# fgnt/pb_bss

Hardware: NVIDIA B200
Metric: EM iterations/s, cACGMM F=513 T=500 D=8 K=3 (100-iteration fit) (higher is better)
Workload: dtype f64

## Files before the change

### pb_bss_b200/csrc/api_cacgmm.cu

```cuda
#include <algorithm>
#include <array>
#include <cstdarg>
#include <cstdlib>
#include <cstring>
#include <map>
#include <mutex>
#include <vector>

#include <cuda.h>

#include "em_kernels.cuh"
#include "em_persistent.cuh"
#include "em_ws.cuh"
#include "em_ls.cuh"
#include "em_sticky.cuh"
#include "prof.cuh"

#ifndef PBB_CTA_FPL
#define PBB_CTA_FPL 2
#endif

namespace pbb {

static thread_local char g_err[512] = "";
// ... 31 lines not shown
  const int k = blockIdx.x;
  __shared__ double red[32];
  double s = 0.0;
  for (int t = threadIdx.x; t < T; t += blockDim.x) s += in[(size_t)k * T + t];
  s = warp_sum(s);
  if ((threadIdx.x & 31) == 0) red[threadIdx.x >> 5] = s;
  __syncthreads();
  if (threadIdx.x == 0) {
    double tot = 0.0;
    for (int i = 0; i < (int)(blockDim.x >> 5); ++i) tot += red[i];
    out[k] = tot / (double)T;
  }
}

__global__ void unit_norm_over_classes_kernel(double* __restrict__ w, int K, int T) {
  const int t = blockIdx.x * blockDim.x + threadIdx.x;
  if (t >= T) return;
  double n = 0.0;
  for (int k = 0; k < K; ++k) n += fabs(w[(size_t)k * T + t]);
  if (n == 0.0) n = 1e-10;
  for (int k = 0; k < K; ++k) w[(size_t)k * T + t] /= n;
}

struct CacgmmWorkspace {
  void* z;
  int zs;
  int* flags;
  int* ticket;
  unsigned long long* phase;
  int* dead;
  double* part;
  double* coef;
  double* ld;
  double* w;
  double* ew;
  double* loglik_part;
  double* aff_stage;
  int* tcount;
  size_t bytes;
};

static int max_chunks(int T) { return (T + 31) / 32; }
constexpr int kMaxOrder = 1 << 20;

static CacgmmWorkspace carve(void* base, int F, int T, int D, int K) {
  CacgmmWorkspace ws;
  const size_t NS = (size_t)D * D;
  size_t off = 0;
  auto take = [&](size_t n) { size_t o = off; off += align_up(n); return o; };
  const int zs = (T + 31) / 32 * 32;
  const size_t nchunks = ((size_t)zs + kStageFrames - 1) / kStageFrames;
  const size_t z_plain = (size_t)F * D * zs * sizeof(double2);
  const size_t z_staged = (size_t)F * nchunks * stage_rows(D % 2 == 0 ? D : D + 1) * kStageFrames * sizeof(double2);
  const size_t o_z = take(z_plain > z_staged ? z_plain : z_staged);
  const size_t o_flags = take((size_t)(F + 1) * sizeof(int) + 16 * sizeof(unsigned long long) + 8);
  const size_t o_dead = take((size_t)F * sizeof(int));
  const size_t o_part = take((size_t)F * max_chunks(T) * K * (NS + 1) * sizeof(double));
  const size_t o_coef = take((size_t)F * (K * NS + 8) * sizeof(double));
  const size_t o_ld = take((size_t)F * (K > 4 ? K : 4) * sizeof(double) + 64);
  const size_t o_w = take((size_t)F * K * sizeof(double));
  const size_t o_ew = take((size_t)F * (K > 4 ? K : 4) * sizeof(double) + 64);
  const size_t o_ll = take((size_t)F * max_chunks(T) * sizeof(double));
  const size_t o_aff = take((size_t)F * K * T * sizeof(double));
  const size_t o_tcount = take((size_t)F * sizeof(int));
  char* b = reinterpret_cast<char*>(base);
  ws.z = b + o_z;
  ws.zs = zs;
  ws.flags = reinterpret_cast<int*>(b + o_flags);
  ws.ticket = ws.flags + F;
  ws.dead = reinterpret_cast<int*>(b + o_dead);
  ws.phase = reinterpret_cast<unsigned long long*>(b + o_flags + (((size_t)(F + 1) * sizeof(int) + 7) / 8) * 8);
  ws.part = reinterpret_cast<double*>(b + o_part);
  ws.coef = reinterpret_cast<double*>(b + o_coef);
  ws.ld = reinterpret_cast<double*>(b + o_ld);
  ws.w = reinterpret_cast<double*>(b + o_w);
  ws.ew = reinterpret_cast<double*>(b + o_ew);
  ws.loglik_part = reinterpret_cast<double*>(b + o_ll);
  ws.aff_stage = reinterpret_cast<double*>(b + o_aff);
// ... 530 lines not shown
  {
    bool h = false;
    const void* alias = nullptr;
    if ((r = classify_pointer(eigenvectors, &alias, &h, "eigenvectors"))) return r;
    eigenvectors = const_cast<void*>(alias);
    if ((r = classify_pointer(eigenvalues, &alias, &h, "eigenvalues"))) return r;
    eigenvalues = static_cast<double*>(const_cast<void*>(alias));
    if ((r = classify_pointer(weight, &alias, &h, "weight"))) return r;
    weight = static_cast<double*>(const_cast<void*>(alias));
  }
  const bool streamed = persistent && y_host && init_aff != nullptr && !(opt->reserved & 2) &&
                        ws.aff_stage != nullptr;
  const bool fast_sm = softmax_fast_ok(D, opt);
  const bool lean_ok = fast_sm && (K - 1) * D * (log10(1.0 / opt->eigenvalue_floor) + 1.0) < 290.0;
  const bool full = saliency != nullptr || activity != nullptr || !lean_ok || init_aff == nullptr;
  const int layout = persistent && use_ls_kernel(D, full) ? 1 : 0;
  std::unique_lock<std::mutex> stream_lock;
  if (streamed) {
    LoadStream* lsm = nullptr;
    if ((r = get_load_stream(&lsm))) return r;
    stream_lock = std::unique_lock<std::mutex>(lsm->mu);
  }
  if (streamed) {
    PBB_CUDA(cudaMemsetAsync(ws.flags, 0, (size_t)(F + 1) * sizeof(int) + 16 * sizeof(unsigned long long) + 8, st));
    PBB_CUDA(cudaMemsetAsync(ws.flags, 0xFF, (size_t)F * sizeof(int), st));
    PBB_CUDA(cudaMemsetAsync(ws.dead, 0, (size_t)F * sizeof(int), st));
    LoadStream* l = nullptr;
    if ((r = get_load_stream(&l))) return r;
    PBB_CUDA(cudaEventRecord(l->fork, st));
    PBB_CUDA(cudaStreamWaitEvent(l->stream, l->fork, 0));
    double* aff_dst = aff_host ? ws.aff_stage : nullptr;
    int* next_bin = reinterpret_cast<int*>(ws.phase + 15);
    int* started = reinterpret_cast<int*>(ws.phase + 14);
    int ctas = 0;
    r = dtype == PBB_C128
            ? launch_stream_load<double2>(y, ws.z, init_aff, aff_dst, F, T, D, K, ws.dead, ws.flags, next_bin, started, &ctas, layout, l->stream)
            : launch_stream_load<float2>(y, ws.z, init_aff, aff_dst, F, T, D, K, ws.dead, ws.flags, next_bin, started, &ctas, layout, l->stream);
    if (r) return r;
    PBB_CUDA(cudaEventRecord(l->join, l->stream));
    if (l->wait_value != nullptr) {
      if (l->wait_value(reinterpret_cast<CUstream>(st), reinterpret_cast<CUdeviceptr>(started), (cuuint32_t)ctas,
                        CU_STREAM_WAIT_VALUE_GEQ) != CUDA_SUCCESS)
        l->wait_value = nullptr;
    }
    if (aff_host) init_aff = ws.aff_stage;
  } else if (persistent)
    r = dtype == PBB_C128 ? launch_normalize_staged<double2>(y, ws.z, F, T, D, ws.dead, layout, st)
// ... 5 lines not shown

  EmArgs a;
  memset(&a, 0, sizeof(a));
  a.z = ws.z; a.zs = ws.zs; a.F = F; a.T = T; a.D = D; a.K = K;
  a.coef = ws.coef; a.ld = ws.ld; a.w = ws.w; a.ew = ws.ew;
  a.activity = activity; a.aff_eps = opt->affiliation_eps;
  a.saliency = saliency; a.part = ws.part;

  UpdArgs u;
  memset(&u, 0, sizeof(u));
  u.F = F; u.T = T; u.D = D; u.K = K;
  u.part = ws.part;
  u.covariance_norm = opt->covariance_norm;
  u.weight_mode = opt->weight_mode;
  u.has_saliency = saliency != nullptr;
  u.eigenvalue_floor = opt->eigenvalue_floor;
  u.evec = reinterpret_cast<double2*>(eigenvectors);
  u.eval = eigenvalues; u.weight = weight;
  u.coef = ws.coef; u.ld = ws.ld; u.ew = ws.ew;
  u.status = status;

  if (persistent) {
    if (!streamed)
      PBB_CUDA(cudaMemsetAsync(ws.flags, 0, (size_t)(F + 1) * sizeof(int) + 16 * sizeof(unsigned long long) + 8, st));
    if (init_aff == nullptr) {
      FromEigArgs fe;
      fe.F = F; fe.D = D; fe.K = K;
      fe.evec = reinterpret_cast<const double2*>(eigenvectors);
      fe.eval = eigenvalues; fe.weight = weight;
      fe.coef = ws.coef; fe.ld = ws.ld; fe.w = ws.w; fe.ew = ws.ew;
      if ((r = launch_from_eig(fe, st))) return r;
    }
    PersistArgs p;
    memset(&p, 0, sizeof(p));
    p.z = ws.z; p.zs = ws.zs; p.F = F; p.T = T;
    p.iterations = opt->iterations;
    p.first_is_m = init_aff != nullptr;
    p.user_model = init_aff == nullptr;
    p.softmax_fast = fast_sm;
    p.aff_in = init_aff; p.saliency = saliency; p.activity = activity;
    p.aff_eps = opt->affiliation_eps; p.eigenvalue_floor = opt->eigenvalue_floor;
    p.covariance_norm = opt->covariance_norm; p.weight_mode = opt->weight_mode;
    p.coef = ws.coef; p.ld = ws.ld; p.w = ws.w; p.ew = ws.ew;
    p.part = ws.part; p.flags = ws.flags; p.ticket = ws.ticket; p.status = status;
    p.phase = ws.phase; p.dead = ws.dead;
    if (streamed) {
      const double bin_bytes = (double)T * D * (dtype == PBB_C128 ? 16.0 : 8.0) + (aff_host ? 8.0 * K * T : 0.0);
// ... 10 lines not shown
        PBB_CUDA(cudaDeviceGetAttribute(&sms, cudaDevAttrMultiProcessorCount, dev));
        int cap = (int)(1.6 * (2 * sms - kLoadReserve));
        if (const char* e = getenv("PBB_ORDER_CAP")) cap = atoi(e);
        if ((r = streamed_order(F, opt->iterations, c, cap < 1 ? 1 : cap, &p.order))) return r;
      }
    }
    bool sticky = false;
    if (D == 8 && !full && !streamed && em_kernel_choice() == 1) {
      if ((r = launch_sticky(p, K, dtype, ws.zs, &sticky, st))) return r;
    }
    if (!sticky) {
      if (!(D == 8 && !full && em_kernel_choice() == 0))
        if ((r = setup_frame_split(&p, ws, F, T, D, K, full ? (D == 8 ? 3 : D == 6 ? 4 : 6) : (D == 4 ? 4 : 2), st)))
          return r;
      if ((r = launch_persist(p, D, K, dtype, full, st))) return r;
    }
    if (streamed) {
      LoadStream* l = nullptr;
      if ((r = get_load_stream(&l))) return r;
      PBB_CUDA(cudaStreamWaitEvent(st, l->join, 0));
    }
#ifdef PBB_PHASE_TIMING
    {
      unsigned long long ph[16];
      cudaStreamSynchronize(st);
      cudaMemcpy(ph, ws.phase, sizeof(ph), cudaMemcpyDeviceToHost);
      fprintf(stderr, "[phase] update of class 0, cycles per task: build %.0f  gauss-jordan %.0f  logdet/tinv %.0f  stores %.0f\n",
              ph[8] / (double)((size_t)F * opt->iterations), ph[9] / (double)((size_t)F * opt->iterations),
              ph[10] / (double)((size_t)F * opt->iterations), ph[11] / (double)((size_t)F * opt->iterations));
      fprintf(stderr, "[phase] producer, cycles per task: ticket->dependency %.0f  model buffer wait %.0f  model issue %.0f  ring refill %.0f\n",
              ph[12] / (double)((size_t)F * opt->iterations), ph[13] / (double)((size_t)F * opt->iterations),
              ph[14] / (double)((size_t)F * opt->iterations), ph[15] / (double)((size_t)F * opt->iterations));
      unsigned long long tot = 0;
      for (int i = 0; i < 8; ++i) tot += ph[i];
      static const char* nm[8] = {"ticket+flag / model wait", "chunk-top / updater busy", "tma-wait", "em-steps", "reduce", "update / S wait", "publish / hand-over", "task-start / updater idle"};
      for (int i = 0; i < 8; ++i) fprintf(stderr, "[phase] %-20s %6.2f%%  %8.0f cycles per task\n", nm[i], 100.0 * ph[i] / (double)tot, ph[i] / (double)((size_t)F * opt->iterations));
    }
#endif
    u.nch = 1;
    u.coef = nullptr;
    return launch_update(u, st);
  }
  int it = 0;
  if (init_aff != nullptr) {
    a.mode = kModeM; a.aff_in = init_aff; a.q_in = nullptr;
    int nch = launch_em(a, dtype, opt->frames_per_block, st);
    if (nch <= 0) return nch ? nch : 1;
    u.nch = nch;
    if ((r = launch_update(u, st))) return r;
// ... 128 lines not shown
  int r;
  if (persistent)
    r = dtype == PBB_C128 ? launch_normalize_staged<double2>(y, ws.z, F, T, D, ws.dead, 0, st)
                          : launch_normalize_staged<float2>(y, ws.z, F, T, D, ws.dead, 0, st);
  else
    r = dtype == PBB_C128 ? launch_normalize<double2>(y, ws.z, F, T, D, 1, ws.zs, st)
                          : launch_normalize<float2>(y, ws.z, F, T, D, 1, ws.zs, st);
  if (r) return r;
  EmArgs a;
  memset(&a, 0, sizeof(a));
  a.z = ws.z; a.zs = ws.zs; a.F = F; a.T = T; a.D = D; a.K = K;
  a.model_kind = 1;
  a.coef = ws.coef; a.ld = ws.ld; a.w = weight; a.ew = ws.ew;
  a.saliency = saliency; a.part = ws.part;
  CwUpdArgs u;
  memset(&u, 0, sizeof(u));
  u.F = F; u.T = T; u.D = D; u.K = K;
  u.part = ws.part; u.weight_mode = weight_mode;
  u.spline.t = spline_t; u.spline.c = spline_c; u.spline.n = spline_n;
  u.spline.max_concentration = max_concentration;
  u.mode = reinterpret_cast<double2*>(mode); u.concentration = concentration; u.weight = weight;
  u.coef = ws.coef; u.ld = ws.ld; u.ew = ws.ew; u.status = status;
  if (persistent) {
    PBB_CUDA(cudaMemsetAsync(ws.flags, 0, (size_t)(F + 1) * sizeof(int) + 16 * sizeof(unsigned long long) + 8, st));
    PersistArgs p;
    memset(&p, 0, sizeof(p));
    p.z = ws.z; p.zs = ws.zs; p.F = F; p.T = T;
    p.iterations = iterations; p.first_is_m = 1; p.user_model = 0; p.softmax_fast = 0;
    p.aff_in = init_aff; p.aff_eps = 0.0; p.weight_mode = weight_mode;
    p.coef = ws.coef; p.ld = ws.ld; p.w = ws.w; p.ew = ws.ew;
    p.part = ws.part; p.flags = ws.flags; p.ticket = ws.ticket; p.status = status; p.phase = ws.phase;
    p.spline = u.spline;
    if ((r = setup_frame_split(&p, ws, F, T, D, K, D == 4 ? 4 : 2, st))) return r;
    if ((r = launch_persist_cw(p, D, K, dtype, st))) return r;
#ifdef PBB_PHASE_TIMING
    {
      unsigned long long ph[16];
      cudaStreamSynchronize(st);
      cudaMemcpy(ph, ws.phase, sizeof(ph), cudaMemcpyDeviceToHost);
      unsigned long long tot = 0;
      for (int i = 0; i < 8; ++i) tot += ph[i];
      static const char* nm[8] = {"flag wait", "chunk top / staging", "tma-wait", "em-steps", "reduce", "update (jacobi)", "publish", "task-start"};
      for (int i = 0; i < 8; ++i) fprintf(stderr, "[phase cw] %-20s %6.2f%%  %8.0f cycles per task\n", nm[i], 100.0 * ph[i] / (double)tot, ph[i] / (double)((size_t)F * iterations));
    }
#endif
    u.nch = 1;
    return launch_cw_update(u, st);
// ... 73 lines not shown
```

### pb_bss_b200/csrc/em_ls.cuh

```cuda
#pragma once
#include "em_ws.cuh"

namespace pbb {

constexpr int kLsWarps = 8;
constexpr int kLsHelpers = 4;
constexpr int kLsThreads = 32 * (kLsWarps + kLsHelpers);
constexpr int kLsUnit = 32;
#ifndef PBB_LS_REGS
#define PBB_LS_REGS 96
#endif
constexpr int kLsRegs = PBB_LS_REGS;
constexpr int kLsHelperRegs = (384 * 80 - 256 * PBB_LS_REGS) / 128;
constexpr int kLsSmemBudget = 113 * 1024;
#ifndef PBB_LS_LEAD
#define PBB_LS_LEAD 0
#endif
#ifndef PBB_LS_HELPERS_FIRST
#define PBB_LS_HELPERS_FIRST 1
#endif

__host__ __device__ constexpr int ls_chan(int h, int r) {
  return h == 0 ? r : (r < 4 ? 4 + r : ((r - 4 + 1) & 3));
}
// ... 521 lines not shown
        int t = 0;
        if (lane == 0) t = atomicAdd(a.ticket, 1);
        t = __shfl_sync(0xffffffffu, t, 0);
        int bin = -1, it = 0;
        if (t < total) {
          if (a.order != nullptr) {
            const int v = __ldcg(a.order + t);
            bin = v & 0xffff;
            it = v >> 16;
          } else {
            decode_ticket(t, F, a.iterations, a.wave_c, bin, it);
          }
        }
        const bool mstep_only = a.first_is_m && it == 0;
        const bool late_z = mstep_only && a.wait_load;
        int dead_bin = 0;
        if (bin >= 0 && a.dead != nullptr && !late_z) dead_bin = __ldcg(a.dead + bin);
        int issued = 0;
        auto issue_chunks = [&](int upto, bool blocking) {
          while (issued < upto) {
            const int st = chunk_cnt % STAGES;
            const uint32_t par = ((chunk_cnt / STAGES) & 1u) ^ 1u;
            if (blocking) {
              mbar_wait_relaxed(&sm.empty[st], par, 100);
            } else {
              uint32_t done;
              asm volatile(
                  "{\n"
                  ".reg .pred p;\n"
                  "mbarrier.test_wait.parity.shared::cta.b64 p, [%1], %2;\n"
                  "selp.u32 %0, 1, 0, p;\n"
                  "}\n"
                  : "=r"(done)
                  : "r"(smem_u32(&sm.empty[st])), "r"(par)
                  : "memory");
              if (!done) break;
            }
            mbar_expect_tx(&sm.full[st], kStageBytes);
            bulk_g2s(&sm.zbuf[st][0][0], zbase + ((size_t)bin * nchunks + issued) * (kStageFrames * 8), kStageBytes,
                     &sm.full[st]);
            ++chunk_cnt;
            ++issued;
          }
        };
#ifdef PBB_PHASE_TIMING
        long long _pt = clock64();
#define PBB_PP(i) do { if (lane == 0) { long long _t = clock64(); atomicAdd(&a.phase[i], (unsigned long long)(_t - _pt)); _pt = _t; } } while (0)
#else
#define PBB_PP(i) do { } while (0)
#endif
        if (bin >= 0 && lane == 0) {
          if (!late_z) issue_chunks(nchunks, false);
          if (mstep_only) {
            if (a.wait_load) while (ld_acquire_gpu(a.flags + bin) < 0) __nanosleep(200);
          } else {
            while (ld_acquire_gpu(a.flags + bin) < it) {
              issue_chunks(nchunks, false);
              __nanosleep(40);
            }
          }
          if (late_z) asm volatile("fence.proxy.async;" ::: "memory");
        }
        __syncwarp();
        PBB_PP(12);
        mbar_wait_relaxed(&sm.model_empty[mb], ((n >> 1) & 1u) ^ 1u, 100);
        PBB_PP(13);
        if (late_z && a.dead != nullptr) dead_bin = __ldcg(a.dead + bin);
        if (bin >= 0 && !mstep_only) {
          constexpr int kPieces = ls_model_doubles(K) / 2;
          constexpr int kRounds = (kPieces + 31) / 32;
          const double2* __restrict__ src = reinterpret_cast<const double2*>(a.coef + (size_t)bin * ls_model_doubles(K));
          double2* __restrict__ dst = reinterpret_cast<double2*>(&sm.model[mb]);
          double2 v[kRounds];
#pragma unroll
          for (int r = 0; r < kRounds; ++r)
            if (lane + 32 * r < kPieces) v[r] = __ldcg(src + lane + 32 * r);
#pragma unroll
          for (int r = 0; r < kRounds; ++r)
            if (lane + 32 * r < kPieces) dst[lane + 32 * r] = v[r];
        }
        if (lane == 0) {
          sm.desc[mb][0] = bin;
          sm.desc[mb][1] = it;
          sm.desc[mb][2] = dead_bin;
        }
        __syncwarp();
        if (lane == 0) mbar_arrive(&sm.model_full[mb]);
        if (bin < 0) break;
        PBB_PP(14);
        if (lane == 0) {
          issue_chunks(nchunks, true);
#if PBB_LS_LEAD
          const unsigned x = chunk_cnt - (unsigned)nchunks;
          mbar_wait_relaxed(&sm.empty[x % STAGES], (x / STAGES) & 1u, 100);
#endif
        }
        __syncwarp();
        PBB_PP(15);
      }
    } else if (hw - 1 < NU) {
      const int u = hw - 1;
      int em[2];
#pragma unroll
      for (int r = 0; r < 2; ++r) {
        const int i = (lane >> 3) + 4 * r, c = lane & 7;
        if (i == c) {
          em[r] = ls_diag_slot(i) | 256;
        } else {
          bool rev = false;
          const int sl = ls_pair_slot(i, c, &rev);
          em[r] = sl | (rev ? 1024 : 512);
        }
      }
#ifdef PBB_PHASE_TIMING
      long long _tp = clock64();
#undef PBB_PH
#define PBB_PH(i) do { if (u == 0 && lane == 0) { long long _t = clock64(); atomicAdd(&a.phase[i], (unsigned long long)(_t - _tp)); _tp = _t; } } while (0)
#endif
#pragma unroll 1
      for (unsigned n = 0;; ++n) {
        mbar_wait_relaxed(&sm.s_full, n & 1u, 100);
        PBB_PH(7);
        const int bin = sm.sdesc[0], it = sm.sdesc[1], dead_bin = sm.sdesc[2];
        if (bin < 0) break;
        const bool last_it = it == a.iterations - 1;
        const int par = n & 1;
        for (int k = u; k < K; k += NU) {
          for (int s = lane; s < NS + 1; s += 32) {
            double v[kLsWarps];
#pragma unroll
            for (int w = 0; w < kLsWarps; ++w) v[w] = sm.Spart[w][k][s];
            sm.S[k][s] = ((v[0] + v[1]) + (v[2] + v[3])) + ((v[4] + v[5]) + (v[6] + v[7]));
          }
        }
        __syncwarp();
        if (lane == 0) mbar_arrive(&sm.s_empty);
        if (last_it) {
          asm volatile("bar.sync 2, %0;" ::"n"(NU * 32) : "memory");
          double* __restrict__ po = a.part + (size_t)bin * K * (NS + 1);
          for (int i = u * 32 + lane; i < K * (NS + 1); i += NU * 32) po[i] = (&sm.S[0][0])[i];
          asm volatile("bar.sync 2, %0;" ::"n"(NU * 32) : "memory");
        } else {
          const bool plain = a.covariance_norm != PBB_NORM_NONE && dead_bin == 0;
          for (int k = u; k < K; k += NU) {
// ... 29 lines not shown
```

### pb_bss_b200/csrc/em_persistent.cuh

```cuda
#pragma once
#include "common.cuh"
#include "em_kernels.cuh"
#include "heig.cuh"

namespace pbb {

#ifdef PBB_PHASE_TIMING
#define PBB_PH(i) do { if (tid == 0) { long long _t = clock64(); atomicAdd(&a.phase[i], (unsigned long long)(_t - _tp)); _tp = _t; } } while (0)
#else
#define PBB_PH(i) do { } while (0)
#endif

struct PersistArgs {
  const void* z;
  int zs;
  int F, T;
  int iterations;
  int first_is_m;
  int user_model;
  int softmax_fast;
  const double* aff_in;
  const double* saliency;
  const uint8_t* activity;
  double aff_eps;
  double eigenvalue_floor;
  int covariance_norm;
  int weight_mode;
  double* coef;
  double* ld;
  double* w;
  double* ew;
  double* part;
  int* flags;
  int* ticket;
  const int* dead;
  int* status;
  CwSpline spline;
  int wave_c;
  int wait_load;
  const int* order;
  unsigned long long* phase;
  int tsplit;
  double* tpart;
  int* tcount;
};

__device__ __forceinline__ uint32_t smem_u32(const void* p) {
  return static_cast<uint32_t>(__cvta_generic_to_shared(p));
}
__device__ __forceinline__ void mbar_init(uint64_t* bar, int count) {
  asm volatile("mbarrier.init.shared::cta.b64 [%0], %1;" ::"r"(smem_u32(bar)), "r"(count) : "memory");
}
__device__ __forceinline__ void mbar_expect_tx(uint64_t* bar, uint32_t bytes) {
  asm volatile("mbarrier.arrive.expect_tx.shared::cta.b64 _, [%0], %1;" ::"r"(smem_u32(bar)), "r"(bytes)
               : "memory");
}
__device__ __forceinline__ void mbar_wait(uint64_t* bar, uint32_t parity) {
  asm volatile(
      "{\n"
      ".reg .pred p;\n"
      "WAIT_%=:\n"
      "mbarrier.try_wait.parity.shared::cta.b64 p, [%0], %1;\n"
      "@p bra DONE_%=;\n"
      "bra WAIT_%=;\n"
      "DONE_%=:\n"
      "}\n" ::"r"(smem_u32(bar)),
      "r"(parity)
      : "memory");
}
__device__ __forceinline__ void bulk_g2s(void* dst, const void* src, uint32_t bytes, uint64_t* bar) {
  asm volatile("cp.async.bulk.shared::cluster.global.mbarrier::complete_tx::bytes [%0], [%1], %2, [%3];" ::"r"(
                   smem_u32(dst)),
               "l"(src), "r"(bytes), "r"(smem_u32(bar))
               : "memory");
}
__device__ __forceinline__ int ld_acquire_gpu(const int* p) {
  int v;
  asm volatile("ld.acquire.gpu.global.s32 %0, [%1];" : "=r"(v) : "l"(p) : "memory");
  return v;
}
__device__ __forceinline__ void st_release_gpu(int* p, int v) {
  asm volatile("st.release.gpu.global.s32 [%0], %1;" ::"l"(p), "r"(v) : "memory");
}
__device__ __forceinline__ double fast_rcp(double x) {
  double r;
  asm("rcp.approx.ftz.f64 %0, %1;" : "=d"(r) : "d"(x));
  double e = fma(-x, r, 1.0);
  r = fma(r, e, r);
  e = fma(-x, r, 1.0);
  r = fma(r, e, r);
  return r;
// ... 455 lines not shown
        done = true;
      }
    }
    if (!done) {
#pragma unroll
      for (int k = 0; k < K; ++k) {
        gam[k] = __ldcg(a.aff_in + ((size_t)bin * K + k) * T + tc);
        invq[k] = 1.0;
      }
    }
    double sal = 1.0;
    if (FULL && a.saliency != nullptr) sal = a.saliency[(size_t)bin * T + tc];
#pragma unroll
    for (int k = 0; k < K; ++k) {
      const double gs = valid ? gam[k] * sal : 0.0;
      const double cw = gs * invq[k];
      sg[k] += gs;
#pragma unroll
      for (int i = 0; i < NSG; ++i) acc[k * NSG + i] = fma(cw, psi[i], acc[k * NSG + i]);
    }
  }
}

template <int D>
__device__ __forceinline__ double warp_hpd_inverse(double2* __restrict__ A, int lane, bool* ok) {
  constexpr int NS = D * D;
  constexpr int PER = (NS + 31) / 32;
  int ri[PER], ci[PER];
  double2 mine[PER];
#pragma unroll
  for (int r = 0; r < PER; ++r) {
    const int idx = lane + 32 * r;
    ri[r] = idx / D;
    ci[r] = idx - ri[r] * D;
    mine[r] = idx < NS ? A[idx] : make_double2(0.0, 0.0);
  }
  double det = 1.0;
  bool good = true;
#pragma unroll 1
  for (int j = 0; j < D; ++j) {
    const double p = A[j * D + j].x;
    good = good && (p > 0.0) && (p < 1e300);
    const double ip = fast_rcp(p);
    det *= p;
#pragma unroll
    for (int r = 0; r < PER; ++r) {
      if (lane + 32 * r < NS) {
        const int i = ri[r], k = ci[r];
// ... 52 lines not shown
        else if (kind == 1) { Ad[2 * (d * D + e)] = v; Ad[2 * (e * D + d)] = v; }
        else { Ad[2 * (d * D + e) + 1] = -v; Ad[2 * (e * D + d) + 1] = v; }
      }
      __syncwarp();
    };
    auto build = [&]() { build_scaled(scale); };
    double tr, tn;
    if (a.covariance_norm == PBB_NORM_NONE) {
      build();
      tr = 0.0;
      for (int d = lane; d < D; d += 32) tr += A[d * D + d].x;
      tr = warp_sum(tr);
      tn = 1.0;
    } else {
      double trs = 0.0;
#pragma unroll
      for (int d = 0; d < D; ++d) trs += Sk[(d >> 1) * (NS / (D / 2)) + (d & 1)];
      tr = trs * scale;
      tn = (double)D / fmax(tr, kTiny);
      build_scaled(scale * tn);
    }
    PBB_PHU(8);
    bool ok;
    const double det = warp_hpd_inverse<D>(A, lane, &ok);
    PBB_PHU(9);
    double ldk = log(det);
    double tinv = 0.0;
#pragma unroll
    for (int d = 0; d < D; ++d) tinv += A[d * D + d].x;
    const bool no_floor = ok && isfinite(tinv) && (tr * tn * tinv * a.eigenvalue_floor < 0.5) &&
                          dead_bin == 0;
    double* __restrict__ co = coef_out != nullptr ? coef_out
                              : LS ? a.coef + (size_t)bin * ls_model_doubles(K) : a.coef + ((size_t)bin * K + k) * NS;
    PBB_PHU(10);
    if (__any_sync(0xffffffffu, bad)) {
      if (lane == 0) atomicMax(a.status, bin + 1);
    }
    if (no_floor) {
      for (int s = lane; s < NS; s += 32) {
        const int pk = tab[s];
        const int d = pk & 255, e = (pk >> 8) & 255, kind = pk >> 16;
        const double2 u = A[d * D + e], v = A[e * D + d];
        const double cv = kind == 0 ? u.x : (kind == 1 ? (u.x + v.x) : -(u.y - v.y));
        if constexpr (LS) ls_store_coef(co, tabE, K, k, s, cv);
        else co[s] = cv;
      }
    } else {
// ... 392 lines not shown
```

### pb_bss_b200/csrc/em_ws.cuh

```cuda
#pragma once
#include "em_persistent.cuh"

namespace pbb {

#ifndef PBB_NO_SOFTMAX_SPLIT
#define PBB_SOFTMAX_SPLIT 1
#endif
#ifndef PBB_WS_LEAD
#define PBB_WS_LEAD 2
#endif
constexpr int kWsStages = 3;
#ifndef PBB_WS_EM_REGS
#define PBB_WS_EM_REGS 208
#endif
constexpr int kWsEmRegs = PBB_WS_EM_REGS;
constexpr int kWsHelperRegs = 256 - PBB_WS_EM_REGS;

__device__ __forceinline__ void mbar_arrive(uint64_t* bar) {
  asm volatile("mbarrier.arrive.shared::cta.b64 _, [%0];" ::"r"(smem_u32(bar)) : "memory");
}

__device__ __forceinline__ void mbar_wait_relaxed(uint64_t* bar, uint32_t parity, unsigned ns) {
  while (true) {
    uint32_t done;
    asm volatile(
        "{\n"
        ".reg .pred p;\n"
        "mbarrier.try_wait.parity.shared::cta.b64 p, [%1], %2;\n"
        "selp.u32 %0, 1, 0, p;\n"
        "}\n"
        : "=r"(done)
        : "r"(smem_u32(bar)), "r"(parity)
        : "memory");
    if (done) break;
    __nanosleep(ns);
  }
}

template <int D, int K, typename CT>
struct WsSmem {
  static constexpr int NS = D * D;
  static constexpr int M = D / 2;
  static constexpr int ROWS = stage_rows(D);
  CT zbuf[kWsStages][ROWS][kStageFrames];
  double2 A[K][NS];
  double2 V[K][NS];
  double coef[2][K][NS];
  double xq[2][M][2 * K][32];
  double cwx[K][64];
  double sgp[2][M][K];
  double S[2][K][NS + 1];
  double lam[K][D];
  double ld[K];
  alignas(16) double ew[2][4];
  int tab[NS];
  int desc[2][4];
  int sdesc[2][4];
  int tlast;
  uint64_t full[kWsStages], empty[kWsStages];
  uint64_t model_full[2], model_empty[2];
// ... 14 lines not shown
  const int nchunks = (zs + kStageFrames - 1) / kStageFrames;
  const int S = a.tsplit > 1 ? a.tsplit : 1;
  const int total = a.iterations * F * S;
  constexpr uint32_t kStageBytes = (uint32_t)(SM::ROWS * kStageFrames * sizeof(CT));

  for (int s = tid; s < NS; s += blockDim.x) sm.tab[s] = slot_pack(D, s);
  if (tid == 0) {
    for (int s = 0; s < kWsStages; ++s) { mbar_init(&sm.full[s], 1); mbar_init(&sm.empty[s], M); }
    for (int s = 0; s < 2; ++s) {
      mbar_init(&sm.model_full[s], 1);
      mbar_init(&sm.model_empty[s], M);
      mbar_init(&sm.s_full[s], M);
      mbar_init(&sm.s_empty[s], NU);
    }
    asm volatile("fence.mbarrier_init.release.cluster;" ::: "memory");
  }
  __syncthreads();

  if (warp < M) {
    asm volatile("setmaxnreg.inc.sync.aligned.u32 %0;" ::"n"(kWsEmRegs));
    const int g = warp;
    unsigned chunk_cnt = 0;
    int buf = 0;
#ifdef PBB_PHASE_TIMING
    long long _tp = clock64();
#endif
#pragma unroll 1
    for (unsigned n = 0;; ++n) {
      const int mb = n & 1;
      mbar_wait(&sm.model_full[mb], (n >> 1) & 1u);
      PBB_PH(0);
      const int bin = sm.desc[mb][0], it = sm.desc[mb][1], part = sm.desc[mb][2];
      const int c0 = part * nchunks / S, c1 = (part + 1) * nchunks / S;
      if (bin < 0) {
        const int sb = n & 1;
        mbar_wait(&sm.s_empty[sb], ((n >> 1) & 1u) ^ 1u);
        if (lane == 0) {
          if (g == 0) sm.sdesc[sb][0] = -1;
          mbar_arrive(&sm.s_full[sb]);
        }
        break;
      }
      const bool mstep_only = a.first_is_m && it == 0;
      double acc[K * NSG];
#pragma unroll
      for (int i = 0; i < K * NSG; ++i) acc[i] = 0.0;
      double sg[K];
#pragma unroll
      for (int k = 0; k < K; ++k) sg[k] = 0.0;
#pragma unroll 1
      for (int c = c0; c < c1; ++c) {
        const int st = chunk_cnt % kWsStages;
        mbar_wait(&sm.full[st], (chunk_cnt / kWsStages) & 1u);
        PBB_PH(2);
        const int t_chunk = c * kStageFrames;
        const int nsteps = (min(kStageFrames, zs - t_chunk)) >> 5;
        if (!mstep_only) {
#ifdef PBB_SOFTMAX_SPLIT
          lean_chunk2_split<D, K, CT>(sm, mb, g, st, nsteps >> 1, lane, a.aff_eps, acc, sg);
          if (nsteps & 1) {
            double sgt[K];
#pragma unroll
            for (int k = 0; k < K; ++k) sgt[k] = 0.0;
            buf = 0;
            lean_chunk<D, K, CT, MODEL, true>(sm, mb, g, st, 1, lane, buf, a.aff_eps, acc, sgt, nsteps - 1);
#pragma unroll
            for (int k = 0; k < K; ++k) sg[k] += g == 0 ? sgt[k] : 0.0;
          }
#else
          lean_chunk2<D, K, CT, MODEL, true>(sm, mb, g, st, nsteps >> 1, lane, buf, a.aff_eps, acc, sg);
          if (nsteps & 1) lean_chunk<D, K, CT, MODEL, true>(sm, mb, g, st, 1, lane, buf, a.aff_eps, acc, sg, nsteps - 1);
#endif
        } else {
          general_chunk<D, K, CT, false>(a, sm, g, bin, st, t_chunk, nsteps, lane, buf, true, true, acc, sg);
        }
        __syncwarp();
// ... 6 lines not shown
#pragma unroll
        for (int k = 0; k < K; ++k) q1[k] = 0.0;
        softmax_product<D, K>(q1, sm.ew[mb], a.aff_eps, gp, cp);
#ifdef PBB_SOFTMAX_SPLIT
        const int npad_lane = (g == 0 && lane >= 32 - (zs - T)) ? 1 : 0;
#else
        const int npad_lane = (lane >= 32 - (zs - T)) ? 1 : 0;
#endif
#pragma unroll
        for (int k = 0; k < K; ++k) sg[k] -= npad_lane ? gp[k] : 0.0;
      }
#ifdef PBB_SOFTMAX_SPLIT
      if (mstep_only && g != 0) {
#pragma unroll
        for (int k = 0; k < K; ++k) sg[k] = 0.0;
      }
#endif
      __syncwarp();
      if (lane == 0) mbar_arrive(&sm.model_empty[mb]);

      warp_reduce_halving<K * NSG>(acc, lane);
      const int sb = n & 1;
      PBB_PH(4);
      mbar_wait(&sm.s_empty[sb], ((n >> 1) & 1u) ^ 1u);
      PBB_PH(5);
      {
        int lo, hi;
        reduce_range<K * NSG>(lane, lo, hi);
#pragma unroll
        for (int j = 0; j < HalvingSizes<K * NSG>::n5; ++j) {
          const int idx = lo + j;
          if (idx < hi) {
            const int k = idx / NSG, i = idx - k * NSG;
            sm.S[sb][k][g * NSG + i] = acc[j];
          }
        }
      }
#pragma unroll
      for (int k = 0; k < K; ++k) {
        const double v = warp_sum(sg[k]);
#ifdef PBB_SOFTMAX_SPLIT
        if (lane == 0) sm.sgp[sb][g][k] = v;
#else
        if (g == 0 && lane == 0) sm.S[sb][k][NS] = v;
#endif
      }
      if (g == 0 && lane == 0) { sm.sdesc[sb][0] = bin; sm.sdesc[sb][1] = it; sm.sdesc[sb][2] = part; }
      __syncwarp();
      if (lane == 0) mbar_arrive(&sm.s_full[sb]);
      PBB_PH(6);
    }
  } else {
    asm volatile("setmaxnreg.dec.sync.aligned.u32 %0;" ::"n"(kWsHelperRegs));
    if (warp == M) {
      const CT* __restrict__ zbase = reinterpret_cast<const CT*>(a.z);
      unsigned chunk_cnt = 0;
#pragma unroll 1
      for (unsigned n = 0;; ++n) {
        const int mb = n & 1;
        int t = 0;
        if (lane == 0) t = atomicAdd(a.ticket, 1);
        t = __shfl_sync(0xffffffffu, t, 0);
        int bin = -1, it = 0, part = 0;
        if (t < total) {
          const int tt = t / S;
          part = t - tt * S;
          if (a.order != nullptr) {
            const int v = __ldcg(a.order + tt);
            bin = v & 0xffff;
            it = v >> 16;
          } else {
            decode_ticket(tt, F, a.iterations, a.wave_c, bin, it);
          }
        }
        const int c0 = part * nchunks / S, ncp = (part + 1) * nchunks / S - c0;
        const bool mstep_only = a.first_is_m && it == 0;
        const bool late_z = mstep_only && a.wait_load;
        int issued = 0;
        auto issue_chunks = [&](int upto, bool blocking) {
          while (issued < upto) {
            const int st = chunk_cnt % kWsStages;
            const uint32_t par = ((chunk_cnt / kWsStages) & 1u) ^ 1u;
            if (blocking) {
              mbar_wait_relaxed(&sm.empty[st], par, 100);
            } else {
              uint32_t done;
              asm volatile(
                  "{\n"
                  ".reg .pred p;\n"
                  "mbarrier.test_wait.parity.shared::cta.b64 p, [%1], %2;\n"
                  "selp.u32 %0, 1, 0, p;\n"
                  "}\n"
                  : "=r"(done)
                  : "r"(smem_u32(&sm.empty[st])), "r"(par)
                  : "memory");
              if (!done) break;
            }
            mbar_expect_tx(&sm.full[st], kStageBytes);
            bulk_g2s(&sm.zbuf[st][0][0], zbase + ((size_t)bin * nchunks + c0 + issued) * (SM::ROWS * kStageFrames),
                     kStageBytes, &sm.full[st]);
            ++chunk_cnt;
            ++issued;
          }
        };
        if (bin >= 0 && lane == 0) {
          if (!late_z) issue_chunks(ncp, false);
          if (mstep_only) {
            if (a.wait_load) while (ld_acquire_gpu(a.flags + bin) < 0) __nanosleep(200);
          } else {
            while (ld_acquire_gpu(a.flags + bin) < it) {
              issue_chunks(ncp, false);
              __nanosleep(40);
            }
          }
          if (late_z) asm volatile("fence.proxy.async;" ::: "memory");
        }
        __syncwarp();
        mbar_wait_relaxed(&sm.model_empty[mb], ((n >> 1) & 1u) ^ 1u, 100);
        if (bin >= 0 && !mstep_only) {
          const double* __restrict__ cf = a.coef + (size_t)bin * K * NS;
          for (int i = lane; i < K * NS; i += 32) (&sm.coef[mb][0][0])[i] = __ldcg(cf + i);
          if (lane < K) {
            const double ldk = __ldcg(a.ld + (size_t)bin * 4 + lane);
            double ldmin = ldk;
#pragma unroll
            for (int j = 0; j < K; ++j) ldmin = fmin(ldmin, __ldcg(a.ld + (size_t)bin * 4 + j));
            const double sgam = __ldcg(a.ew + (size_t)bin * 4 + lane);
            const double wk = a.weight_mode == PBB_WEIGHT_CONST ? 1.0 / K : sgam / (double)T;
            sm.ew[mb][lane] = wk * exp(ldmin - ldk);
          }
        }
        if (lane == 0) { sm.desc[mb][0] = bin; sm.desc[mb][1] = it; sm.desc[mb][2] = part; }
        __syncwarp();
        if (lane == 0) mbar_arrive(&sm.model_full[mb]);
        if (bin < 0) break;
        if (lane == 0) {
          issue_chunks(ncp, true);
          const unsigned x = chunk_cnt - (unsigned)(ncp >= PBB_WS_LEAD + 1 ? PBB_WS_LEAD + 1 : ncp);
          mbar_wait_relaxed(&sm.empty[x % kWsStages], (x / kWsStages) & 1u, 100);
        }
        __syncwarp();
      }
    } else if (warp - M - 1 < NU) {
      const int u = warp - M - 1;
#ifdef PBB_PHASE_TIMING
      long long _tp = clock64();
#undef PBB_PH
#define PBB_PH(i) do { if (u == 0 && lane == 0) { long long _t = clock64(); atomicAdd(&a.phase[i], (unsigned long long)(_t - _tp)); _tp = _t; } } while (0)
#endif
#pragma unroll 1
      for (unsigned n = 0;; ++n) {
        const int sb = n & 1;
        mbar_wait_relaxed(&sm.s_full[sb], (n >> 1) & 1u, 100);
        PBB_PH(7);
        const int bin = sm.sdesc[sb][0], it = sm.sdesc[sb][1];
        if (bin < 0) break;
        const bool last_it = it == a.iterations - 1;
#ifdef PBB_SOFTMAX_SPLIT
        for (int k = u; k < K; k += NU)
          if (lane == 0)
            sm.S[sb][k][NS] = (sm.sgp[sb][0][k] + sm.sgp[sb][1][k]) + (sm.sgp[sb][2][k] + sm.sgp[sb][3][k]);
        __syncwarp();
        if (last_it && S == 1) asm volatile("bar.sync 2, %0;" ::"n"(NU * 32) : "memory");
#endif
        if (S > 1) {
          const int part = sm.sdesc[sb][2];
          constexpr int kRow = K * (NS + 1);
          double* __restrict__ tp = a.tpart + ((size_t)bin * S + part) * kRow;
          for (int k = u; k < K; k += NU)
            for (int i = lane; i < NS + 1; i += 32) __stcg(tp + k * (NS + 1) + i, sm.S[sb][k][i]);
          __threadfence();
          asm volatile("bar.sync 2, %0;" ::"n"(NU * 32) : "memory");
          if (u == 0 && lane == 0) {
            const int old = atomicAdd(a.tcount + bin, 1);
            __threadfence();
            sm.tlast = (old + 1 == (it + 1) * S);
          }
          asm volatile("bar.sync 2, %0;" ::"n"(NU * 32) : "memory");
          if (!sm.tlast) {
// ... 35 lines not shown
```

Baseline: 43600.

## Use hinted mbarrier waits, backoff flag polling, and block 8x8 HPD inverse

Replaces the sleep-based mbarrier polling in helper warps with try_wait carrying a suspend-time hint, so threads park in hardware instead of spinning with fixed nanosleeps. The load-flag poll now backs off exponentially instead of sleeping a fixed interval. It also adds a specialised 2x2-block Gauss-Jordan inverse for D=8 that ping-pongs between two shared buffers, plus trip-count instrumentation that only compiles under the phase-timing flag. Long hint values could delay wakeups in helper warps if the hardware honours the full suspend window.

```diff
diff --git a/pb_bss_b200/csrc/api_cacgmm.cu b/pb_bss_b200/csrc/api_cacgmm.cu
--- a/pb_bss_b200/csrc/api_cacgmm.cu
+++ b/pb_bss_b200/csrc/api_cacgmm.cu
@@ -77,6 +77,7 @@
   for (int k = 0; k < K; ++k) w[(size_t)k * T + t] /= n;
 }
 
+constexpr int kPhaseSlots = 32;
 struct CacgmmWorkspace {
   void* z;
   int zs;
@@ -108,7 +109,7 @@
   const size_t z_plain = (size_t)F * D * zs * sizeof(double2);
   const size_t z_staged = (size_t)F * nchunks * stage_rows(D % 2 == 0 ? D : D + 1) * kStageFrames * sizeof(double2);
   const size_t o_z = take(z_plain > z_staged ? z_plain : z_staged);
-  const size_t o_flags = take((size_t)(F + 1) * sizeof(int) + 16 * sizeof(unsigned long long) + 8);
+  const size_t o_flags = take((size_t)(F + 1) * sizeof(int) + kPhaseSlots * sizeof(unsigned long long) + 8);
   const size_t o_dead = take((size_t)F * sizeof(int));
   const size_t o_part = take((size_t)F * max_chunks(T) * K * (NS + 1) * sizeof(double));
   const size_t o_coef = take((size_t)F * (K * NS + 8) * sizeof(double));
@@ -685,7 +686,7 @@
     stream_lock = std::unique_lock<std::mutex>(lsm->mu);
   }
   if (streamed) {
-    PBB_CUDA(cudaMemsetAsync(ws.flags, 0, (size_t)(F + 1) * sizeof(int) + 16 * sizeof(unsigned long long) + 8, st));
+    PBB_CUDA(cudaMemsetAsync(ws.flags, 0, (size_t)(F + 1) * sizeof(int) + kPhaseSlots * sizeof(unsigned long long) + 8, st));
     PBB_CUDA(cudaMemsetAsync(ws.flags, 0xFF, (size_t)F * sizeof(int), st));
     PBB_CUDA(cudaMemsetAsync(ws.dead, 0, (size_t)F * sizeof(int), st));
     LoadStream* l = nullptr;
@@ -737,7 +738,7 @@
 
   if (persistent) {
     if (!streamed)
-      PBB_CUDA(cudaMemsetAsync(ws.flags, 0, (size_t)(F + 1) * sizeof(int) + 16 * sizeof(unsigned long long) + 8, st));
+      PBB_CUDA(cudaMemsetAsync(ws.flags, 0, (size_t)(F + 1) * sizeof(int) + kPhaseSlots * sizeof(unsigned long long) + 8, st));
     if (init_aff == nullptr) {
       FromEigArgs fe;
       fe.F = F; fe.D = D; fe.K = K;
@@ -794,9 +795,14 @@
     }
 #ifdef PBB_PHASE_TIMING
     {
-      unsigned long long ph[16];
+      unsigned long long ph[kPhaseSlots];
       cudaStreamSynchronize(st);
       cudaMemcpy(ph, ws.phase, sizeof(ph), cudaMemcpyDeviceToHost);
+      static const char* tn[7] = {"EM model", "EM ring", "EM S buffer", "producer ring slot", "producer flag poll",
+                                  "producer model buffer", "updater S buffer"};
+      for (int i = 0; i < 7; ++i)
+        fprintf(stderr, "[trips] %-22s %10llu  %8.2f per task\n", tn[i], ph[kPhaseTrip + i],
+                ph[kPhaseTrip + i] / (double)((size_t)F * opt->iterations));
       fprintf(stderr, "[phase] update of class 0, cycles per task: build %.0f  gauss-jordan %.0f  logdet/tinv %.0f  stores %.0f\n",
               ph[8] / (double)((size_t)F * opt->iterations), ph[9] / (double)((size_t)F * opt->iterations),
               ph[10] / (double)((size_t)F * opt->iterations), ph[11] / (double)((size_t)F * opt->iterations));
@@ -971,7 +977,7 @@
   u.mode = reinterpret_cast<double2*>(mode); u.concentration = concentration; u.weight = weight;
   u.coef = ws.coef; u.ld = ws.ld; u.ew = ws.ew; u.status = status;
   if (persistent) {
-    PBB_CUDA(cudaMemsetAsync(ws.flags, 0, (size_t)(F + 1) * sizeof(int) + 16 * sizeof(unsigned long long) + 8, st));
+    PBB_CUDA(cudaMemsetAsync(ws.flags, 0, (size_t)(F + 1) * sizeof(int) + kPhaseSlots * sizeof(unsigned long long) + 8, st));
     PersistArgs p;
     memset(&p, 0, sizeof(p));
     p.z = ws.z; p.zs = ws.zs; p.F = F; p.T = T;
diff --git a/pb_bss_b200/csrc/em_ls.cuh b/pb_bss_b200/csrc/em_ls.cuh
--- a/pb_bss_b200/csrc/em_ls.cuh
+++ b/pb_bss_b200/csrc/em_ls.cuh
@@ -567,7 +567,7 @@
             const int st = chunk_cnt % STAGES;
             const uint32_t par = ((chunk_cnt / STAGES) & 1u) ^ 1u;
             if (blocking) {
-              mbar_wait_relaxed(&sm.empty[st], par, 100);
+              mbar_wait(&sm.empty[st], par, kWaitHintHelper);
             } else {
               uint32_t done;
               asm volatile(
@@ -608,7 +608,7 @@
         }
         __syncwarp();
         PBB_PP(12);
-        mbar_wait_relaxed(&sm.model_empty[mb], ((n >> 1) & 1u) ^ 1u, 100);
+        mbar_wait(&sm.model_empty[mb], ((n >> 1) & 1u) ^ 1u, kWaitHintHelper);
         PBB_PP(13);
         if (late_z && a.dead != nullptr) dead_bin = __ldcg(a.dead + bin);
         if (bin >= 0 && !mstep_only) {
@@ -637,7 +637,7 @@
           issue_chunks(nchunks, true);
 #if PBB_LS_LEAD
           const unsigned x = chunk_cnt - (unsigned)nchunks;
-          mbar_wait_relaxed(&sm.empty[x % STAGES], (x / STAGES) & 1u, 100);
+          mbar_wait(&sm.empty[x % STAGES], (x / STAGES) & 1u, kWaitHintHelper);
 #endif
         }
         __syncwarp();
@@ -664,7 +664,7 @@
 #endif
 #pragma unroll 1
       for (unsigned n = 0;; ++n) {
-        mbar_wait_relaxed(&sm.s_full, n & 1u, 100);
+        mbar_wait(&sm.s_full, n & 1u, kWaitHintHelper);
         PBB_PH(7);
         const int bin = sm.sdesc[0], it = sm.sdesc[1], dead_bin = sm.sdesc[2];
         if (bin < 0) break;
diff --git a/pb_bss_b200/csrc/em_persistent.cuh b/pb_bss_b200/csrc/em_persistent.cuh
--- a/pb_bss_b200/csrc/em_persistent.cuh
+++ b/pb_bss_b200/csrc/em_persistent.cuh
@@ -7,8 +7,15 @@
 
 #ifdef PBB_PHASE_TIMING
 #define PBB_PH(i) do { if (tid == 0) { long long _t = clock64(); atomicAdd(&a.phase[i], (unsigned long long)(_t - _tp)); _tp = _t; } } while (0)
+constexpr int kPhaseTrip = 16;
+#define PBB_TRIPS_DECL(n) unsigned long long _trips[n] = {}; constexpr int _ntrips = n
+#define PBB_TRIP(j, e) (_trips[j] += (e))
+#define PBB_TRIPS_FLUSH(base) do { if (lane == 0) for (int _j = 0; _j < _ntrips; ++_j) atomicAdd(&a.phase[(base) + _j], _trips[_j]); } while (0)
 #else
 #define PBB_PH(i) do { } while (0)
+#define PBB_TRIPS_DECL(n) do { } while (0)
+#define PBB_TRIP(j, e) ((void)(e))
+#define PBB_TRIPS_FLUSH(base) do { } while (0)
 #endif
 
 struct PersistArgs {
@@ -55,18 +62,25 @@
   asm volatile("mbarrier.arrive.expect_tx.shared::cta.b64 _, [%0], %1;" ::"r"(smem_u32(bar)), "r"(bytes)
                : "memory");
 }
-__device__ __forceinline__ void mbar_wait(uint64_t* bar, uint32_t parity) {
+__device__ __forceinline__ bool mbar_try_wait(uint64_t* bar, uint32_t parity, uint32_t hint_ns) {
+  uint32_t done;
   asm volatile(
       "{\n"
       ".reg .pred p;\n"
-      "WAIT_%=:\n"
-      "mbarrier.try_wait.parity.shared::cta.b64 p, [%0], %1;\n"
-      "@p bra DONE_%=;\n"
-      "bra WAIT_%=;\n"
-      "DONE_%=:\n"
-      "}\n" ::"r"(smem_u32(bar)),
-      "r"(parity)
+      "mbarrier.try_wait.parity.shared::cta.b64 p, [%1], %2, %3;\n"
+      "selp.u32 %0, 1, 0, p;\n"
+      "}\n"
+      : "=r"(done)
+      : "r"(smem_u32(bar)), "r"(parity), "r"(hint_ns)
       : "memory");
+  return done != 0;
+}
+constexpr uint32_t kWaitHintEm = 2000;
+constexpr uint32_t kWaitHintHelper = 1000000;
+__device__ __forceinline__ unsigned mbar_wait(uint64_t* bar, uint32_t parity, uint32_t hint_ns = kWaitHintEm) {
+  unsigned trips = 1;
+  while (!mbar_try_wait(bar, parity, hint_ns)) ++trips;
+  return trips;
 }
 __device__ __forceinline__ void bulk_g2s(void* dst, const void* src, uint32_t bytes, uint64_t* bar) {
   asm volatile("cp.async.bulk.shared::cluster.global.mbarrier::complete_tx::bytes [%0], [%1], %2, [%3];" ::"r"(
@@ -568,8 +582,67 @@
   }
 }
 
+__device__ __forceinline__ double2 cfma(double2 y, double2 b, double2 acc) {
+  return make_double2(fma(y.x, b.x, fma(-y.y, b.y, acc.x)), fma(y.x, b.y, fma(y.y, b.x, acc.y)));
+}
+
+__device__ __forceinline__ double warp_hpd_inverse8(double2* __restrict__ A, double2* __restrict__ W, int lane,
+                                                    bool* ok) {
+  constexpr int D = 8;
+  const int i = lane >> 2, c = lane & 3, I = i >> 1, r0 = i & 1;
+  double2 m0 = A[i * D + 2 * c], m1 = A[i * D + 2 * c + 1];
+  double det = 1.0;
+  bool good = true;
+#pragma unroll
+  for (int j = 0; j < 4; ++j) {
+    const double2* __restrict__ src = (j & 1) ? W : A;
+    double2* __restrict__ dst = (j & 1) ? A : W;
+    const int p = 2 * j;
+    const double pa = src[p * D + p].x, pd = src[(p + 1) * D + p + 1].x;
+    const double2 pb = src[p * D + p + 1];
+    const double dp = fma(pa, pd, -fma(pb.x, pb.x, pb.y * pb.y));
+    good = good && (pa > 0.0) && (dp > 0.0) && (pa < 1e300) && (dp < 1e300);
+    det *= dp;
+    const double r = fast_rcp(dp);
+    const double ia = pd * r, id = pa * r;
+    const double2 ib = make_double2(-pb.x * r, -pb.y * r);
+    double2 y0, y1;
+    if (I == j) {
+      y0 = r0 ? make_double2(ib.x, -ib.y) : make_double2(ia, 0.0);
+      y1 = r0 ? make_double2(id, 0.0) : ib;
+    } else {
+      const double2 x0 = src[i * D + p], x1 = src[i * D + p + 1];
+      y0 = make_double2(fma(x0.x, ia, fma(x1.x, ib.x, x1.y * ib.y)), fma(x0.y, ia, fma(x1.y, ib.x, -x1.x * ib.y)));
+      y1 = make_double2(fma(x0.x, ib.x, fma(-x0.y, ib.y, x1.x * id)), fma(x0.x, ib.y, fma(x0.y, ib.x, x1.y * id)));
+    }
+    if (c == j) {
+      m0 = I == j ? y0 : make_double2(-y0.x, -y0.y);
+      m1 = I == j ? y1 : make_double2(-y1.x, -y1.y);
+    } else {
+      const double2 b00 = src[p * D + 2 * c], b01 = src[p * D + 2 * c + 1];
+      const double2 b10 = src[(p + 1) * D + 2 * c], b11 = src[(p + 1) * D + 2 * c + 1];
+      if (I == j) {
+        m0 = make_double2(0.0, 0.0);
+        m1 = make_double2(0.0, 0.0);
+      } else {
+        y0 = make_double2(-y0.x, -y0.y);
+        y1 = make_double2(-y1.x, -y1.y);
+      }
+      m0 = cfma(y1, b10, cfma(y0, b00, m0));
+      m1 = cfma(y1, b11, cfma(y0, b01, m1));
+    }
+    dst[i * D + 2 * c] = m0;
+    dst[i * D + 2 * c + 1] = m1;
+    __syncwarp();
+  }
+  *ok = good;
+  return det;
+}
+
 template <int D>
-__device__ __forceinline__ double warp_hpd_inverse(double2* __restrict__ A, int lane, bool* ok) {
+__device__ __forceinline__ double warp_hpd_inverse(double2* __restrict__ A, double2* __restrict__ W, int lane,
+                                                   bool* ok) {
+  if constexpr (D == 8) return warp_hpd_inverse8(A, W, lane, ok);
   constexpr int NS = D * D;
   constexpr int PER = (NS + 31) / 32;
   int ri[PER], ci[PER];
@@ -668,7 +741,7 @@
     }
     PBB_PHU(8);
     bool ok;
-    const double det = warp_hpd_inverse<D>(A, lane, &ok);
+    const double det = warp_hpd_inverse<D>(A, V, lane, &ok);
     PBB_PHU(9);
     double ldk = log(det);
     double tinv = 0.0;
diff --git a/pb_bss_b200/csrc/em_ws.cuh b/pb_bss_b200/csrc/em_ws.cuh
--- a/pb_bss_b200/csrc/em_ws.cuh
+++ b/pb_bss_b200/csrc/em_ws.cuh
@@ -20,22 +20,7 @@
   asm volatile("mbarrier.arrive.shared::cta.b64 _, [%0];" ::"r"(smem_u32(bar)) : "memory");
 }
 
-__device__ __forceinline__ void mbar_wait_relaxed(uint64_t* bar, uint32_t parity, unsigned ns) {
-  while (true) {
-    uint32_t done;
-    asm volatile(
-        "{\n"
-        ".reg .pred p;\n"
-        "mbarrier.try_wait.parity.shared::cta.b64 p, [%1], %2;\n"
-        "selp.u32 %0, 1, 0, p;\n"
-        "}\n"
-        : "=r"(done)
-        : "r"(smem_u32(bar)), "r"(parity)
-        : "memory");
-    if (done) break;
-    __nanosleep(ns);
-  }
-}
+constexpr unsigned kFlagPollMinNs = 32, kFlagPollMaxNs = 256;
 
 template <int D, int K, typename CT>
 struct WsSmem {
@@ -96,23 +81,25 @@
     const int g = warp;
     unsigned chunk_cnt = 0;
     int buf = 0;
+    PBB_TRIPS_DECL(3);
 #ifdef PBB_PHASE_TIMING
     long long _tp = clock64();
 #endif
 #pragma unroll 1
     for (unsigned n = 0;; ++n) {
       const int mb = n & 1;
-      mbar_wait(&sm.model_full[mb], (n >> 1) & 1u);
+      PBB_TRIP(0, mbar_wait(&sm.model_full[mb], (n >> 1) & 1u));
       PBB_PH(0);
       const int bin = sm.desc[mb][0], it = sm.desc[mb][1], part = sm.desc[mb][2];
       const int c0 = part * nchunks / S, c1 = (part + 1) * nchunks / S;
       if (bin < 0) {
         const int sb = n & 1;
-        mbar_wait(&sm.s_empty[sb], ((n >> 1) & 1u) ^ 1u);
+        PBB_TRIP(2, mbar_wait(&sm.s_empty[sb], ((n >> 1) & 1u) ^ 1u));
         if (lane == 0) {
           if (g == 0) sm.sdesc[sb][0] = -1;
           mbar_arrive(&sm.s_full[sb]);
         }
+        PBB_TRIPS_FLUSH(kPhaseTrip);
         break;
       }
       const bool mstep_only = a.first_is_m && it == 0;
@@ -125,7 +112,7 @@
 #pragma unroll 1
       for (int c = c0; c < c1; ++c) {
         const int st = chunk_cnt % kWsStages;
-        mbar_wait(&sm.full[st], (chunk_cnt / kWsStages) & 1u);
+        PBB_TRIP(1, mbar_wait(&sm.full[st], (chunk_cnt / kWsStages) & 1u));
         PBB_PH(2);
         const int t_chunk = c * kStageFrames;
         const int nsteps = (min(kStageFrames, zs - t_chunk)) >> 5;
@@ -178,7 +165,7 @@
       warp_reduce_halving<K * NSG>(acc, lane);
       const int sb = n & 1;
       PBB_PH(4);
-      mbar_wait(&sm.s_empty[sb], ((n >> 1) & 1u) ^ 1u);
+      PBB_TRIP(2, mbar_wait(&sm.s_empty[sb], ((n >> 1) & 1u) ^ 1u));
       PBB_PH(5);
       {
         int lo, hi;
@@ -211,6 +198,7 @@
     if (warp == M) {
       const CT* __restrict__ zbase = reinterpret_cast<const CT*>(a.z);
       unsigned chunk_cnt = 0;
+      PBB_TRIPS_DECL(3);
 #pragma unroll 1
       for (unsigned n = 0;; ++n) {
         const int mb = n & 1;
@@ -238,7 +226,7 @@
             const int st = chunk_cnt % kWsStages;
             const uint32_t par = ((chunk_cnt / kWsStages) & 1u) ^ 1u;
             if (blocking) {
-              mbar_wait_relaxed(&sm.empty[st], par, 100);
+              PBB_TRIP(0, mbar_wait(&sm.empty[st], par, kWaitHintHelper));
             } else {
               uint32_t done;
               asm volatile(
@@ -264,15 +252,16 @@
           if (mstep_only) {
             if (a.wait_load) while (ld_acquire_gpu(a.flags + bin) < 0) __nanosleep(200);
           } else {
-            while (ld_acquire_gpu(a.flags + bin) < it) {
+            for (unsigned ns = kFlagPollMinNs; ld_acquire_gpu(a.flags + bin) < it; ns = min(2 * ns, kFlagPollMaxNs)) {
+              PBB_TRIP(1, 1u);
               issue_chunks(ncp, false);
-              __nanosleep(40);
+              __nanosleep(ns);
             }
           }
           if (late_z) asm volatile("fence.proxy.async;" ::: "memory");
         }
         __syncwarp();
-        mbar_wait_relaxed(&sm.model_empty[mb], ((n >> 1) & 1u) ^ 1u, 100);
+        PBB_TRIP(2, mbar_wait(&sm.model_empty[mb], ((n >> 1) & 1u) ^ 1u, kWaitHintHelper));
         if (bin >= 0 && !mstep_only) {
           const double* __restrict__ cf = a.coef + (size_t)bin * K * NS;
           for (int i = lane; i < K * NS; i += 32) (&sm.coef[mb][0][0])[i] = __ldcg(cf + i);
@@ -289,16 +278,20 @@
         if (lane == 0) { sm.desc[mb][0] = bin; sm.desc[mb][1] = it; sm.desc[mb][2] = part; }
         __syncwarp();
         if (lane == 0) mbar_arrive(&sm.model_full[mb]);
-        if (bin < 0) break;
+        if (bin < 0) {
+          PBB_TRIPS_FLUSH(kPhaseTrip + 3);
+          break;
+        }
         if (lane == 0) {
           issue_chunks(ncp, true);
           const unsigned x = chunk_cnt - (unsigned)(ncp >= PBB_WS_LEAD + 1 ? PBB_WS_LEAD + 1 : ncp);
-          mbar_wait_relaxed(&sm.empty[x % kWsStages], (x / kWsStages) & 1u, 100);
+          PBB_TRIP(0, mbar_wait(&sm.empty[x % kWsStages], (x / kWsStages) & 1u, kWaitHintHelper));
         }
         __syncwarp();
       }
     } else if (warp - M - 1 < NU) {
       const int u = warp - M - 1;
+      PBB_TRIPS_DECL(1);
 #ifdef PBB_PHASE_TIMING
       long long _tp = clock64();
 #undef PBB_PH
@@ -307,10 +300,13 @@
 #pragma unroll 1
       for (unsigned n = 0;; ++n) {
         const int sb = n & 1;
-        mbar_wait_relaxed(&sm.s_full[sb], (n >> 1) & 1u, 100);
+        PBB_TRIP(0, mbar_wait(&sm.s_full[sb], (n >> 1) & 1u, kWaitHintHelper));
         PBB_PH(7);
         const int bin = sm.sdesc[sb][0], it = sm.sdesc[sb][1];
-        if (bin < 0) break;
+        if (bin < 0) {
+          PBB_TRIPS_FLUSH(kPhaseTrip + 6);
+          break;
+        }
         const bool last_it = it == a.iterations - 1;
 #ifdef PBB_SOFTMAX_SPLIT
         for (int k = u; k < K; k += NU)
```

Result: no change. 44000 (median of 6 runs) (+0.9%).
